# skynavga/orion-sdr

Measured on AMD Instinct MI355X. Metric: Msamples/s through WBFM demod chain (NCO+decim+FM discrim) at 1/2/4/8 MI355X, higher is better.
Workload: dtype f32; 1 GPU; C2 WBFM chain: Rotator(-f_off) -> FirDecimator(10e6, 8, 200e3, 79e3; 127 taps) -> FmQuadratureDemod(1.25e6, 75e3, 15e3) -> FirLowpass(1.25e6, 15e3, 10e3; 125 taps); channels_per_gpu=1, parallelism=channel-sharded x1, no data-path collective

## Files before the change

### orion-sdr_amd/csrc/k_wbfm.hip

```cpp
#include <algorithm>
#include <cstdlib>

#include "iir.hpp"
#include "kernels.hpp"
#include "poly.hpp"

namespace orion {
namespace {

__device__ __forceinline__ void lds_order() { asm volatile("" ::: "memory"); }

constexpr int NT = 256;
constexpr int T = kWbfmT;
constexpr int M = kWbfmM;
constexpr int Q = kWbfmQ;
using PW = Poly<M, Q, T, NT>;
static_assert(PW::NS == kWbfmNS, "staging size");
constexpr int KP = (PW::NS + 2 * NT - 1) / (2 * NT);
static_assert(2 * NT * (KP - 1) + 2 * NT - 1 >= PW::NS - 1, "staging coverage");


template <int R>
struct Fw {
  static constexpr int TW = 64 * R;
  static constexpr int NEW = M * TW;
  static constexpr int KL = NEW / 128;
  static constexpr int LR = TW + Q + 2;
  static constexpr int WIN = (R + Q) / 2;
  static constexpr int LDS_F2 = M * LR;
  static_assert(LR % 16 == 2, "row pitch = 2 mod 16 (phase-scattered b64 stores)");
  static_assert((R % 2) == 0 && NEW <= kWbfmNS, "phasor table covers the tile");
};


__device__ __forceinline__ float wave_shr1(float v, float first) {
  return __int_as_float(__builtin_amdgcn_update_dpp(__float_as_int(first), __float_as_int(v), 0x138,
                                                    0xf, 0xf, false));
}

template <int R, bool A16, bool CLAMP>
__device__ __forceinline__ void front2_load(const f2* __restrict__ x, long long n, long long porg,
                                            int l, f2 (&v)[Fw<R>::KL][2]) {
  const long long B = porg + 8 * Q;
  const f2* __restrict__ xb;
  int lo = 0, hi = 0;
  if constexpr (CLAMP) {
    constexpr long long kSat = 1LL << 30;
    lo = static_cast<int>(max(-B, -kSat));
    hi = static_cast<int>(min(max((n - 2 - B) & ~1LL, -kSat), kSat));
    xb = x + B;
  } else {
    xb = x + min(max(B, 0LL), (n - Fw<R>::NEW) & ~1LL);
  }
#pragma unroll
  for (int k = 0; k < Fw<R>::KL; ++k) {
    const int o = CLAMP ? min(max(2 * l + 128 * k, lo), hi) : 2 * l + 128 * k;
    if constexpr (A16) {
      const f4 w = __builtin_nontemporal_load(reinterpret_cast<const f4*>(xb + o));
      v[k][0] = f2{w.x, w.y};
      v[k][1] = f2{w.z, w.w};
    } else {
      v[k][0] = xb[o];
      v[k][1] = xb[o + 1];
    }
  }
}

template <int R>
__device__ __forceinline__ void front2_phase(const f4 (&w)[Fw<R>::WIN], const float (&t)[Q], f2 (&d)[R]) {
#pragma unroll
  for (int h = 0; h < Fw<R>::WIN; ++h) {
    const f2 w0 = f2{w[h].x, w[h].y}, w1 = f2{w[h].z, w[h].w};
#pragma unroll
    for (int r = 0; r < R; ++r) {
      const int q0 = r + Q - 2 * h, q1 = r + Q - 2 * h - 1;
      if (q0 >= 0 && q0 < Q) d[r] = fma2(splat2(t[q0]), w0, d[r]);
      if (q1 >= 0 && q1 < Q) d[r] = fma2(splat2(t[q1]), w1, d[r]);
    }
  }
}

template <int R>
__device__ __forceinline__ void front2_window(const f2* __restrict__ U, int l, int c, f4 (&w)[Fw<R>::WIN]) {
  const f4* row = reinterpret_cast<const f4*>(U + c * Fw<R>::LR + R * l);
#pragma unroll
  for (int h = 0; h < Fw<R>::WIN; ++h) w[h] = row[h];
}
__device__ __forceinline__ void front2_taps(const float* __restrict__ g, int c, float (&t)[Q]) {
#pragma unroll
  for (int q = 0; q < Q; ++q) t[q] = g[c * Q + q];
}

template <int R>
__device__ __forceinline__ void front2_decim(const f2* __restrict__ U, int l, const float* __restrict__ g,
                                             f2 (&d)[R]) {
#pragma unroll
  for (int r = 0; r < R; ++r) d[r] = f2{0.0f, 0.0f};
#pragma unroll 1
  for (int c = 0; c < M; ++c) {
    f4 w[Fw<R>::WIN];
    float t[Q];
    front2_window<R>(U, l, c, w);
    front2_taps(g, c, t);
    front2_phase<R>(w, t, d);
  }
}

template <int R, bool A16, bool CLAMP = false>
__global__ __launch_bounds__(64, R <= 2 ? 3 : 2) void k_wbfm_front2(const WbfmArgs a, const WbfmFrontConst C,
                                                    long long L, int wpc) {
  using G = Fw<R>;
  __shared__ __attribute__((aligned(16))) f2 U[G::LDS_F2];
  const int l = threadIdx.x;
  const int ch = blockIdx.x / wpc;
  const long long A = static_cast<long long>(blockIdx.x - ch * wpc) * L;
  const long long B = min(A + L, a.n_dec);
  if (A >= B) return;
// ... 356 lines not shown
template <int N>
struct Geo {
  static constexpr int L = 128 * N;
  static constexpr int NH = L / 2;
  static constexpr int CH = NH / 64;
  static_assert((CH & (CH - 1)) == 0 && CH >= 8, "chunk a power of two");
  __host__ __device__ static constexpr int pslot(int e) { return e + e / CH; }
  static constexpr int PSlots = pslot(NH + PB) + 1;
};

__device__ __forceinline__ void st_agent(uint32_t* p, uint32_t v) {
  __hip_atomic_store(p, v, __ATOMIC_RELAXED, __HIP_MEMORY_SCOPE_AGENT);
}
__device__ __forceinline__ uint32_t ld_agent(const uint32_t* p) {
  return __hip_atomic_load(p, __ATOMIC_RELAXED, __HIP_MEMORY_SCOPE_AGENT);
}
__device__ __forceinline__ void stores_done() { __builtin_amdgcn_s_waitcnt(0x0F70); }
__device__ __forceinline__ void publish(uint32_t* flag, uint32_t epoch, int l) {
  stores_done();
  if (l == 0) st_agent(flag, epoch);
}
__device__ __forceinline__ void wait_for(const uint32_t* flag, uint32_t epoch, int* err, uint32_t spin) {
  for (uint32_t it = 0; it < spin; ++it) {
    if (ld_agent(flag) == epoch) {
      asm volatile("" ::: "memory");
      return;
    }
    __builtin_amdgcn_s_sleep(4);
  }
  if ((threadIdx.x & 63) == 0) __hip_atomic_store(err, 1, __ATOMIC_RELAXED, __HIP_MEMORY_SCOPE_SYSTEM);
}
__device__ __forceinline__ double u2d(uint32_t lo, uint32_t hi) {
  return __longlong_as_double(static_cast<long long>((static_cast<unsigned long long>(hi) << 32) | lo));
}
}

struct FuTile {
  const WbfmArgs& a;
  const WbfmFrontConst& C;
  f2* U;
  float* Phi;
  const float* Gt;
  const f2* xc;
  const f2* hc;
  const f2* tabc;
  int ch, l, s0, s1;
  f2 corr;
  bool first;
};
struct FuPrefetch {
  const f2* xl;
  long long nl, porg;
  bool on;
};

namespace g8 {
constexpr int PCH = 91;
constexpr int LRS = 2 * PCH;
constexpr int LDS_F2 = M * LRS;
__host__ __device__ constexpr int pchunk(int c) { return 5 * (c >> 2) + (c & 3); }
__host__ __device__ constexpr int slot(int i) { return 2 * pchunk(i >> 1) + (i & 1); }
static_assert(slot(fu::G::TW + Q) < LRS && pchunk(fu::G::TW / 2) == 80, "row geometry");
__device__ __forceinline__ int group(int l) {
  const int i = l & 31;
  const bool a = i < 4 || (i >= 12 && i < 16) || (i >= 20 && i < 28);
  return (l >> 5) * 2 + (a ? 0 : 1);
}
__device__ __forceinline__ int prev_lane(int l) {
  const int row = l >> 4, lp = l & 15;
  return row == 0 ? 47 + lp : row == 2 ? lp : row == 1 ? 32 + lp : 16 + lp;
}
__device__ __forceinline__ int first_out(int l) {
  const int row = l >> 4;
  return 8 * (l & 15) + 2 * (row == 0 ? 0 : row == 2 ? 1 : row == 1 ? 2 : 3);
}
template <bool FIRST, bool ORD>
__device__ __forceinline__ void phase(const f2* __restrict__ U, int c, int lp, const float* __restrict__ Gt,
                                      f2 (&d)[8]) {
  const f4* __restrict__ row = reinterpret_cast<const f4*>(U + c * LRS) + 5 * lp;
  const f4* __restrict__ tq = reinterpret_cast<const f4*>(Gt + c * Q);
  f4 w[12];
  float t[Q];
  if constexpr (ORD) {
#pragma unroll
    for (int q4 = Q / 4 - 1; q4 >= 0; --q4) {
      const f4 u = tq[q4];
      t[4 * q4] = u.x;
      t[4 * q4 + 1] = u.y;
      t[4 * q4 + 2] = u.z;
      t[4 * q4 + 3] = u.w;
    }
#pragma unroll
    for (int h = 0; h < 12; ++h) w[h] = row[5 * (h >> 2) + (h & 3)];
  } else {
#pragma unroll
    for (int h = 0; h < 12; ++h) w[h] = row[5 * (h >> 2) + (h & 3)];
#pragma unroll
    for (int q4 = 0; q4 < Q / 4; ++q4) {
      const f4 u = tq[q4];
      t[4 * q4] = u.x;
      t[4 * q4 + 1] = u.y;
      t[4 * q4 + 2] = u.z;
      t[4 * q4 + 3] = u.w;
    }
  }
#pragma unroll
  for (int qi = 0; qi < Q; ++qi) {
    const int q = ORD ? Q - 1 - qi : qi;
#pragma unroll
    for (int r = 0; r < 8; ++r) {
      const int m = r + Q - q;
      const f4& wc = w[m >> 1];
      const f2 xv = (m & 1) ? f2{wc.z, wc.w} : f2{wc.x, wc.y};
      if (FIRST && qi == 0) {
        d[r] = splat2(t[q]) * xv;
      } else {
        d[r] = fma2(splat2(t[q]), xv, d[r]);
      }
    }
  }
}
}

template <bool A16, bool CLAMP>
__device__ __forceinline__ void fu_tile8(const FuTile& T, int n, long long porg, long long jd0,
                                         const f2 (&ph)[8][2], f2 (&v)[8][2], const FuPrefetch& pf, f2 Sv,
                                         f2& carry, float* __restrict__ phit, int svi) {
  using G = fu::G;
  f2* __restrict__ U = T.U;
  const int l = T.l;
  const int hc = l & 7, hh = l >> 3;
  f4 hw = f4{0, 0, 0, 0};
  f2 hq = f2{0, 0};
  if (n > 0) {
    hw = *reinterpret_cast<const f4*>(U + hc * g8::LRS + 2 * (80 + g8::pchunk(hh)));
    if (l < 7) hq = U[(l + 1) * g8::LRS + g8::slot(G::TW + Q)];
  }
  const bool bnd = porg < 0 || porg + 8LL * (G::TW + Q) > T.a.n;
#pragma unroll
  for (int k = 0; k < G::KL; ++k) {
    U[T.s0 + 20 * k] = cmul_rot_pk(v[k][0], ph[k][0]);
    U[T.s1 + 20 * k] = cmul_rot_pk(v[k][1], ph[k][1]);
    if (k % 4 == 3) asm volatile("" ::: "memory");
  }
  asm volatile("" ::: "memory");
  if (n > 0) {
    const f2 y0 = cmul(f2{hw.x, hw.y}, T.corr), y1 = cmul(f2{hw.z, hw.w}, T.corr);
    *reinterpret_cast<f4*>(U + hc * g8::LRS + 2 * g8::pchunk(hh)) = f4{y0.x, y0.y, y1.x, y1.y};
    if (l < 7) U[(l + 1) * g8::LRS + g8::slot(Q)] = cmul(hq, T.corr);
  }
  front2_load<2, A16, CLAMP>(pf.xl, pf.nl, pf.porg, l, v);
  if (bnd) {
    lds_order();
#pragma unroll 1
    for (int p = (n == 0 ? 0 : 8 * Q) + l; p < 8 * (G::TW + Q); p += 64) {
      const long long Pp = porg + p;
      if (!CLAMP || Pp < 0 || Pp >= T.a.n || p < 8 * Q) {
        const int c = (-p) & 7;
        U[c * g8::LRS + g8::slot((p + c) / 8)] = cmul_rot(load_hist(T.xc, T.a.n, T.hc, kWbfmHist, Pp), T.tabc[p]);
      }
    }
  }
  lds_order();
  const int g = g8::group(l), lp = l & 15;
  f2 d[8];
  g8::phase<true, true>(U, 2 * g, lp, T.Gt, d);
  asm volatile("" ::: "memory");
  g8::phase<false, true>(U, 2 * g + 1, lp, T.Gt, d);
  f2 K[4];
#pragma unroll
  for (int i = 0; i < 4; ++i) {
    const auto sx = __builtin_amdgcn_permlane16_swap(__float_as_uint(d[i].x), __float_as_uint(d[i + 4].x), false, false);
    const auto sy = __builtin_amdgcn_permlane16_swap(__float_as_uint(d[i].y), __float_as_uint(d[i + 4].y), false, false);
    K[i] = f2{__uint_as_float(sx[0]), __uint_as_float(sy[0])} + f2{__uint_as_float(sx[1]), __uint_as_float(sy[1])};
  }
  f2 F[2];
#pragma unroll
  for (int i = 0; i < 2; ++i) {
    const auto sx = __builtin_amdgcn_permlane32_swap(__float_as_uint(K[i].x), __float_as_uint(K[i + 2].x), false, false);
    const auto sy = __builtin_amdgcn_permlane32_swap(__float_as_uint(K[i].y), __float_as_uint(K[i + 2].y), false, false);
    F[i] = f2{__uint_as_float(sx[0]), __uint_as_float(sy[0])} + f2{__uint_as_float(sx[1]), __uint_as_float(sy[1])};
  }
  const f2 S = f2{__int_as_float(__builtin_amdgcn_readlane(__float_as_int(Sv.x), svi)),
                  __int_as_float(__builtin_amdgcn_readlane(__float_as_int(Sv.y), svi))};
  F[0] = cmul(F[0], S);
  F[1] = cmul(F[1], S);
  if (n == 0 && !T.first) {
    f2 acc = f2{0.0f, 0.0f};
#pragma unroll
    for (int t2 = 0; t2 < 2; ++t2) {
      const int k = 2 * l + t2, c = k & 7, q = k >> 3;
      acc = fma2(splat2(T.Gt[c * Q + q]), U[c * g8::LRS + g8::slot(15 - q)], acc);
    }
#pragma unroll
    for (int off = 32; off >= 1; off >>= 1)
      acc += f2{__shfl_xor(acc.x, off, 64), __shfl_xor(acc.y, off, 64)};
    carry = cmul(acc, S);
  }
  const int src = g8::prev_lane(l);
  f2 pv = f2{__shfl(F[1].x, src, 64), __shfl(F[1].y, src, 64)};
  if (l == 0) pv = carry;
  const int j0 = g8::first_out(l);
  *reinterpret_cast<f2*>(phit + j0) = f2{fm_disc_pk_rcp(F[0], pv, T.C.k), fm_disc_pk_rcp(F[1], F[0], T.C.k)};
  carry = f2{__int_as_float(__builtin_amdgcn_readlane(__float_as_int(F[1].x), 63)),
             __int_as_float(__builtin_amdgcn_readlane(__float_as_int(F[1].y), 63))};
  const WbfmArgs& a = T.a;
  if (jd0 <= a.n_dec - 1 && a.n_dec - 1 < jd0 + G::TW) {
    const int rl = static_cast<int>(a.n_dec - 1 - jd0);
    float* co = a.carry_out + T.ch * kWbfmCarry;
#pragma unroll
    for (int r = 0; r < 2; ++r)
      if (j0 + r == rl) {
        co[4] = F[r].x;
        co[5] = F[r].y;
        co[6] = 0.0f;
        co[7] = 0.0f;
      }
#pragma unroll
    for (int t2 = 0; t2 < kWbfmHist / 64; ++t2) {
      const int t = l + 64 * t2;
      a.hist_out[T.ch * kWbfmHist + t] = load_hist(T.xc, a.n, T.hc, kWbfmHist, a.n - kWbfmHist + t);
    }
  }
}

struct FuRange {
  int r, ch, wl;
  long long A, B;
  int Lr;
  bool first, last;
};
__device__ __forceinline__ FuPrefetch fu_origin(const WbfmArgs& a, const FuRange& g) {
  const bool tiny = a.n < 2;
  FuPrefetch p;
  p.xl = tiny ? a.hist_in + g.ch * kWbfmHist : a.x + g.ch * a.x_stride;
  p.nl = tiny ? kWbfmHist : a.n;
  p.porg = 8LL * (g.A - Q);
  p.on = true;
  return p;
}

constexpr int kSegPrioQ16 = 9;
namespace sg {
constexpr int NS = 8;
using Y = fu::Geo<NS>;
constexpr int L = Y::L;
constexpr int CH = Y::CH;
constexpr int WBytes = (Y::PSlots * 8 > L * 4) ? Y::PSlots * 8 : L * 4;
constexpr int kSegSlot = kSeg4Slot;

__device__ __forceinline__ double uni(double v) {
  const long long b = __double_as_longlong(v);
  const int lo = __builtin_amdgcn_readfirstlane(static_cast<int>(b));
  const int hi = __builtin_amdgcn_readfirstlane(static_cast<int>(b >> 32));
  return __longlong_as_double((static_cast<long long>(hi) << 32) | static_cast<unsigned int>(lo));
}

typedef const __attribute__((address_space(4))) double* cmat_t;
__device__ __forceinline__ cmat_t mats_of(const WbfmFusedConst& Bc) {
  const double* p = Bc.mats;
  asm volatile("" : "+s"(p));
  return (cmat_t)(p);
}
template <int S>
__device__ __forceinline__ void matvec_c(cmat_t M, const double (&x)[S], double (&y)[S]) {
#pragma unroll
  for (int i = 0; i < S; ++i)
#pragma unroll
    for (int j = 0; j < S; ++j) y[i] = __builtin_fma(M[i * S + j], x[j], y[i]);
}
__device__ __forceinline__ void iir16(const WbfmFusedConst& Bc, const float* __restrict__ Phi, int l,
                                      const double (&sw)[4], f2 (&xs)[CH], f2 (&ef)[4], double (&send)[4]) {
#pragma unroll
  for (int i = 0; i < CH; i += 4) {
    const f4 u = *reinterpret_cast<const f4*>(Phi + 16 * l + i);
    const f4 w = *reinterpret_cast<const f4*>(Phi + 16 * l + 8 + i);
    xs[i] = f2{u.x, w.x};
    xs[i + 1] = f2{u.y, w.y};
    xs[i + 2] = f2{u.z, w.z};
    xs[i + 3] = f2{u.w, w.w};
  }
  lds_order();
  const Biquad2 bq{splat2(Bc.b0), splat2(Bc.b1), splat2(Bc.b2), splat2(Bc.a1), splat2(Bc.a2)};
  f2 z[4] = {f2{0, 0}, f2{0, 0}, f2{0, 0}, f2{0, 0}};
#pragma unroll
  for (int i = 0; i < CH; ++i) (void)bq.lp4(z, xs[i]);
  double zE[4], q[4];
#pragma unroll
  for (int k = 0; k < 4; ++k) {
    zE[k] = z[k].x;
    q[k] = z[k].y;
  }
  const cmat_t pw = mats_of(Bc);
  matvec_c<4>(pw, zE, q);
  {
    double f[4] = {0, 0, 0, 0};
    matvec_c<4>(pw + 16, sw, f);
#pragma unroll
    for (int k = 0; k < 4; ++k) q[k] += l == 0 ? f[k] : 0.0;
  }
#pragma unroll 1
  for (int st = 0; st < 6; ++st) {
    const int dd = 1 << st;
    double o[4];
#pragma unroll
    for (int k = 0; k < 4; ++k) o[k] = __shfl_up(q[k], dd, 64);
    if (l >= dd) matvec_c<4>(pw + (st + 1) * 16, o, q);
  }
#pragma unroll
  for (int k = 0; k < 4; ++k) {
    const long long b = __double_as_longlong(q[k]);
    const int lo = __builtin_amdgcn_readlane(static_cast<int>(b), 63);
    const int hi = __builtin_amdgcn_readlane(static_cast<int>(b >> 32), 63);
    send[k] = __longlong_as_double((static_cast<long long>(hi) << 32) | static_cast<unsigned int>(lo));
  }
  double eE[4], eO[4];
#pragma unroll
  for (int k = 0; k < 4; ++k) {
    const double o = __shfl_up(q[k], 1, 64);
    eE[k] = l == 0 ? sw[k] : o;
    eO[k] = zE[k];
  }
  matvec_c<4>(pw, eE, eO);
#pragma unroll
  for (int k = 0; k < 4; ++k) ef[k] = f2{static_cast<float>(eE[k]), static_cast<float>(eO[k])};
}

__device__ __forceinline__ void zs_only16(const WbfmFusedConst& Bc, const float* Phi, float* tmp, int l,
                                          double (&sw)[4], float (&hout)[2]) {
  const double zero[4] = {0, 0, 0, 0};
  f2 xs[CH], ef[4];
  iir16(Bc, Phi, l, zero, xs, ef, sw);
  const Biquad2 bq{splat2(Bc.b0), splat2(Bc.b1), splat2(Bc.b2), splat2(Bc.a1), splat2(Bc.a2)};
  int to = 16 * (l - 56);
  asm volatile("" : "+v"(to));
  float* __restrict__ tl = tmp + to;
#pragma unroll
  for (int i = 0; i < CH; ++i) {
    const f2 f = bq.lp4(ef, xs[i]);
    if (l >= 56) {
      tl[i] = f.x;
      tl[8 + i] = f.y;
    }
  }
  lds_order();
  hout[0] = tmp[l];
  hout[1] = tmp[l + 64];
  lds_order();
}

__host__ __device__ constexpr int pe(int e) { return e + ((e >> 7) << 3); }
constexpr int kFpN = pe(128 + 1024 + 16) + 8;
#ifndef ORION_WBFM_EXACT_FIR
#define ORION_WBFM_EXACT_FIR 0
#endif
#if ORION_WBFM_EXACT_FIR
__host__ __device__ constexpr int pf(int e) { return e + 4 * (e >> 6); }
constexpr int kTxOff = pf(128 + 1024 + 16) * 4;
#else
constexpr int kTxOff = 2 * kFpN * 2;
#endif
static_assert(kTxOff % 16 == 0 && kTxOff + 128 * 4 <= WBytes, "f planes + exact history fit the sub-range region");
typedef _Float16 h8 __attribute__((ext_vector_type(8)));
__device__ __forceinline__ _Float16 hi16(float x) { return static_cast<_Float16>(x); }
__device__ __forceinline__ _Float16 lo16(float x, _Float16 h) { return static_cast<_Float16>(x - static_cast<float>(h)); }

template <int CTRL>
__device__ __forceinline__ float dpp_max(float v) {
  return fmaxf(v, __int_as_float(__builtin_amdgcn_update_dpp(0, __float_as_int(v), CTRL, 0xf, 0xf, false)));
}
__device__ __forceinline__ float wave_max(float v) {
  v = dpp_max<0xB1>(v);
  v = dpp_max<0x4E>(v);
  v = dpp_max<0x141>(v);
  v = dpp_max<0x140>(v);
  const auto r16 = __builtin_amdgcn_permlane16_swap(__float_as_uint(v), __float_as_uint(v), false, false);
  v = fmaxf(__uint_as_float(r16[0]), __uint_as_float(r16[1]));
  const auto r32 = __builtin_amdgcn_permlane32_swap(__float_as_uint(v), __float_as_uint(v), false, false);
  return fmaxf(__uint_as_float(r32[0]), __uint_as_float(r32[1]));
}

__device__ __forceinline__ void publish_end(const WbfmArgs& a, int r, const double (&sw)[4], const float (&hist)[2],
                                            int l) {
  uint32_t* slot = a.hand + static_cast<long long>(r) * kSegSlot;
  if (l < 8) {
    const int kk = l >> 1;
    const double v8 = kk == 0 ? sw[0] : kk == 1 ? sw[1] : kk == 2 ? sw[2] : sw[3];
    const unsigned long long b = static_cast<unsigned long long>(__double_as_longlong(v8));
    fu::st_agent(slot + 2 + l, (l & 1) ? static_cast<uint32_t>(b >> 32) : static_cast<uint32_t>(b));
  }
  fu::st_agent(slot + 16 + l, __float_as_uint(hist[0]));
  fu::st_agent(slot + 16 + 64 + l, __float_as_uint(hist[1]));
  fu::publish(a.flags + 3LL * r, a.epoch, l);
}

__device__ __forceinline__ void back(const WbfmArgs& a, const WbfmFusedConst& Bc, int ch, long long A0, int Lr,
                                     bool chan_last, const float* Phi, void* Pv, const uint32_t* __restrict__ Aw,
                                     int l, double (&sw)[4], float (&hist)[2], int publish_r = -1,
                                     int trace_r = -1) {
  const Biquad2 bq{splat2(Bc.b0), splat2(Bc.b1), splat2(Bc.b2), splat2(Bc.a1), splat2(Bc.a2)};
  _Float16* __restrict__ Fh = static_cast<_Float16*>(Pv);
  _Float16* __restrict__ Fl = Fh + kFpN;
  float* __restrict__ Tx = reinterpret_cast<float*>(static_cast<unsigned char*>(Pv) + kTxOff);
  f2 xs[CH];
  {
    f2 ef[4];
    double send[4];
    iir16(Bc, Phi, l, sw, xs, ef, send);
    if (trace_r >= 0) fu::trace(a, trace_r, 10);
    const int jl = Lr - 1;
    float cap[4] = {0, 0, 0, 0};
    bool have = false;
#pragma unroll
    for (int i = 0; i < CH; ++i) {
      const int j = 16 * l + i;
      const f2 f = bq.lp4(ef, xs[i]);
      xs[i] = f2{j < Lr ? f.x : 0.0f, j + 8 < Lr ? f.y : 0.0f};
      const int te = j - Lr + 128;
      if (te >= 0 && te < 128) Tx[te] = f.x;
      if (te + 8 >= 0 && te + 8 < 128) Tx[te + 8] = f.y;
      if (chan_last) {
        if (j == jl) {
#pragma unroll
          for (int k = 0; k < 4; ++k) cap[k] = ef[k].x;
          have = true;
        }
        if (j + 8 == jl) {
#pragma unroll
          for (int k = 0; k < 4; ++k) cap[k] = ef[k].y;
          have = true;
        }
      }
    }
    if (have) {
      float* co = a.carry_out + ch * kWbfmCarry;
#pragma unroll
      for (int k = 0; k < 4; ++k) co[k] = cap[k];
    }
    const int lend = Lr >= L ? 63 : max(0, (Lr >> 4) - 1);
#pragma unroll
    for (int k = 0; k < 4; ++k)
      sw[k] = static_cast<double>(__int_as_float(__builtin_amdgcn_readlane(__float_as_int(ef[k].y), lend)));
  }
  if (Lr < 128) {
#pragma unroll
    for (int r2 = 0; r2 < 2; ++r2) {
      const int t = l + 64 * r2 - Lr;
      if (t >= 0) Tx[t] = hist[r2];
    }
  }
#if ORION_WBFM_EXACT_FIR
  const int sf = 0;
  {
    float* __restrict__ Fp = static_cast<float*>(Pv);
    const int e0 = pf(128 + 16 * l);
    *reinterpret_cast<f4*>(Fp + e0) = f4{xs[0].x, xs[1].x, xs[2].x, xs[3].x};
    *reinterpret_cast<f4*>(Fp + e0 + 4) = f4{xs[4].x, xs[5].x, xs[6].x, xs[7].x};
    *reinterpret_cast<f4*>(Fp + e0 + 8) = f4{xs[0].y, xs[1].y, xs[2].y, xs[3].y};
    *reinterpret_cast<f4*>(Fp + e0 + 12) = f4{xs[4].y, xs[5].y, xs[6].y, xs[7].y};
#pragma unroll
    for (int r2 = 0; r2 < 2; ++r2) Fp[pf(l + 64 * r2)] = hist[r2];
    if (l < 4) *reinterpret_cast<f4*>(Fp + pf(128 + 1024 + 4 * l)) = f4{0, 0, 0, 0};
  }
#else
  float mx = fmaxf(fabsf(hist[0]), fabsf(hist[1]));
#pragma unroll
  for (int i = 0; i < CH; ++i) mx = fmaxf(mx, fmaxf(fabsf(xs[i].x), fabsf(xs[i].y)));
  mx = wave_max(mx);
  const int sf = __builtin_amdgcn_readfirstlane(min(100, 15 - __builtin_amdgcn_frexp_expf(mx)));
  {
    typedef _Float16 h2 __attribute__((ext_vector_type(2)));
    const int e0 = pe(128 + 16 * l);
#pragma unroll
    for (int i = 0; i < CH; i += 2) {
      h2 eh, el, oh, ol;
#pragma unroll
      for (int u = 0; u < 2; ++u) {
        const float fe = __builtin_amdgcn_ldexpf(xs[i + u].x, sf), fo = __builtin_amdgcn_ldexpf(xs[i + u].y, sf);
        eh[u] = hi16(fe);
        el[u] = lo16(fe, eh[u]);
        oh[u] = hi16(fo);
        ol[u] = lo16(fo, oh[u]);
      }
      *reinterpret_cast<h2*>(Fh + e0 + i) = eh;
      *reinterpret_cast<h2*>(Fl + e0 + i) = el;
      *reinterpret_cast<h2*>(Fh + e0 + 8 + i) = oh;
      *reinterpret_cast<h2*>(Fl + e0 + 8 + i) = ol;
    }
  }
#pragma unroll
  for (int r2 = 0; r2 < 2; ++r2) {
    const int e = pe(l + 64 * r2);
    const float x = __builtin_amdgcn_ldexpf(hist[r2], sf);
    const _Float16 h = hi16(x);
    Fh[e] = h;
    Fl[e] = lo16(x, h);
  }
  if (l < 2) {
    const h8 z = h8{0, 0, 0, 0, 0, 0, 0, 0};
    *reinterpret_cast<h8*>(Fh + pe(128 + 1024 + 8 * l)) = z;
    *reinterpret_cast<h8*>(Fl + pe(128 + 1024 + 8 * l)) = z;
  }
#endif
  lds_order();
#pragma unroll
  for (int r2 = 0; r2 < 2; ++r2) hist[r2] = Tx[l + 64 * r2];
  if (publish_r >= 0) publish_end(a, publish_r, sw, hist, l);
  if (chan_last) {
#pragma unroll
    for (int r2 = 0; r2 < 2; ++r2) a.carry_out[ch * kWbfmCarry + 8 + l + 64 * r2] = hist[r2];
  }
  if (trace_r >= 0) fu::trace(a, trace_r, 11);
  {
    const int J = l & 15, kg = l >> 4;
    typedef float f4v __attribute__((ext_vector_type(4)));
    f4v acc[4];
#pragma unroll
    for (int g = 0; g < 4; ++g) acc[g] = f4v{0.0f, 0.0f, 0.0f, 0.0f};
#if ORION_WBFM_EXACT_FIR
    {
      const float* __restrict__ Fp = static_cast<const float*>(Pv);
      const float* __restrict__ At = reinterpret_cast<const float*>(Aw);
      const int I = l & 15;
#pragma unroll 4
      for (int st = 0; st < 40; ++st) {
        const float av = At[I - 4 * st - kg + 159];
        const int p = pf(16 * J + 4 * st + kg);
        float b[4];
#pragma unroll
        for (int g = 0; g < 4; ++g) b[g] = Fp[p + 272 * g];
#pragma unroll
        for (int g = 0; g < 4; ++g) acc[g] = __builtin_amdgcn_mfma_f32_16x16x4f32(av, b[g], acc[g], 0, 0, 0);
      }
    }
#else
    const int I = l & 15;
#pragma unroll 1
    for (int st = 0; st < 5; ++st) {
      h8 ah, al;
      {
        const int o = 32 * st + 8 * kg - I - 1, p = o & 1;
// ... 4 lines not shown
        ah = __builtin_bit_cast(h8, vh);
        al = __builtin_bit_cast(h8, vl);
      }
      h8 bh[4], bl[4];
#pragma unroll
      for (int g = 0; g < 4; ++g) {
        const int e = pe(256 * g + 16 * J + 32 * st + 8 * kg);
        bh[g] = *reinterpret_cast<const h8*>(Fh + e);
        bl[g] = *reinterpret_cast<const h8*>(Fl + e);
      }
#pragma unroll
      for (int g = 0; g < 4; ++g) acc[g] = __builtin_amdgcn_mfma_f32_16x16x32_f16(ah, bh[g], acc[g], 0, 0, 0);
#pragma unroll
      for (int g = 0; g < 4; ++g) acc[g] = __builtin_amdgcn_mfma_f32_16x16x32_f16(ah, bl[g], acc[g], 0, 0, 0);
#pragma unroll
      for (int g = 0; g < 4; ++g) acc[g] = __builtin_amdgcn_mfma_f32_16x16x32_f16(al, bh[g], acc[g], 0, 0, 0);
      asm volatile("" ::: "memory");
      if (trace_r >= 0 && st == 0) fu::trace(a, trace_r, 13);
    }
#endif
    if (trace_r >= 0) fu::trace(a, trace_r, 14);
    float* __restrict__ y = a.y + ch * a.y_stride + A0;
    const float ys = __builtin_amdgcn_ldexpf(Bc.tscale, -sf);
    if (Lr == L && (reinterpret_cast<uintptr_t>(y) & 15) == 0) {
#pragma unroll
      for (int g = 0; g < 4; ++g)
        *reinterpret_cast<float4*>(y + 256 * g + 16 * J + 4 * kg) =
            float4{acc[g][0] * ys, acc[g][1] * ys, acc[g][2] * ys, acc[g][3] * ys};
    } else {
#pragma unroll
      for (int g = 0; g < 4; ++g)
#pragma unroll
        for (int r = 0; r < 4; ++r) {
          const int j = 256 * g + 16 * J + 4 * kg + r;
          if (j < Lr) y[j] = acc[g][r] * ys;
        }
    }
  }
  lds_order();
  if (trace_r >= 0) fu::trace(a, trace_r, 12);
}

}

template <bool A16, bool CLAMP>
__global__ __launch_bounds__(64, 2) void k_wbfm_seg(const WbfmArgs a, const WbfmFrontConst C,
                                                    const WbfmFusedConst Bc, int spc, int S) {
  using G = fu::G;
  constexpr int TW = G::TW;
  __shared__ __attribute__((aligned(16))) f2 U[g8::LDS_F2];
  __shared__ __attribute__((aligned(16))) unsigned char wreg[sg::WBytes];
  __shared__ __attribute__((aligned(16))) float Gt[128];
  __shared__ __attribute__((aligned(16))) uint32_t Aw[kAudFragBytes / 4];
  float* Phi = reinterpret_cast<float*>(wreg);
  f2* P = reinterpret_cast<f2*>(wreg);
  const int l = threadIdx.x & 63;
  Gt[l] = C.g[l];
  Gt[l + 64] = C.g[l + 64];
  {
    const uint32_t* __restrict__ aw = static_cast<const uint32_t*>(a.afrag);
#pragma unroll
    for (int i = 0; i < kAudFragBytes / 4 / 64; ++i) Aw[l + 64 * i] = aw[l + 64 * i];
  }
  FuRange g;
  g.r = blockIdx.x;
  g.ch = g.r / spc;
  g.wl = g.r - g.ch * spc;
  g.A = static_cast<long long>(g.wl) * S;
  g.B = min(g.A + S, a.n_dec);
  g.Lr = static_cast<int>(g.B - g.A);
  g.first = g.wl == 0;
  g.last = g.B == a.n_dec;
  const bool late = blockIdx.x >= (gridDim.x >> 1);
  const int nsub = (g.Lr + sg::L - 1) / sg::L;
  const int ntiles = nsub * sg::NS;
  uint32_t* const myslot = a.hand + static_cast<long long>(g.r) * sg::kSegSlot;
  fu::trace(a, g.r, 0);

  const FuPrefetch org = fu_origin(a, g);
  f2 va[G::KL][2];
  front2_load<2, A16, CLAMP>(org.xl, org.nl, org.porg, l, va);
  const f2* __restrict__ tabc = a.tab + static_cast<long long>(g.ch) * kWbfmNS;
  const f2* __restrict__ xc = a.x + g.ch * a.x_stride;
  const f2* __restrict__ hc = a.hist_in + g.ch * kWbfmHist;
  const f2 cn = tabc[G::NEW];
  const int c0 = (-2 * l) & 7, c1 = (-2 * l - 1) & 7;
  const FuTile T{a, C, U, Phi, Gt, xc, hc, tabc, g.ch, l, c0 * g8::LRS + g8::slot((8 * Q + 2 * l + c0) / 8),
                 c1 * g8::LRS + g8::slot((8 * Q + 2 * l + 1 + c1) / 8), f2{cn.x, -cn.y}, g.first};
  long long porg = org.porg;
  {
    const long long P0 = porg + 2 * l;
    const long long hi = (org.nl & ~1LL) - 2;
    const long long Pc = P0 < 0 ? 0 : (P0 > hi ? hi : P0);
    const f2 x0 = org.xl[Pc], x1 = org.xl[Pc + 1];
    const f4 th = *reinterpret_cast<const f4*>(tabc + 2 * l);
    U[c0 * g8::LRS + g8::slot((2 * l + c0) / 8)] = cmul_rot(x0, f2{th.x, th.y});
    U[c1 * g8::LRS + g8::slot((2 * l + 1 + c1) / 8)] = cmul_rot(x1, f2{th.z, th.w});
  }
  {
    const long long Pm = max(porg - (l & 7), 0LL);
    const f2 xm = xc[Pm];
    const f2 tc = tabc[l & 7];
    if (!g.first && l >= 1 && l < 8) U[l * g8::LRS] = cmul_rot(xm, f2{tc.x, -tc.y});
  }
  f2 Sv = f2{0, 0};
  f2 carry = f2{0.0f, 0.0f};
  if (g.first) {
    const float* ci = a.carry_in + g.ch * kWbfmCarry;
    carry = f2{ci[4], ci[5]};
  }
  double sw[4] = {0, 0, 0, 0};
  float hist[2] = {0, 0};
  const FuPrefetch dummy{org.xl, org.nl, -8LL * Q, true};

#pragma unroll 1
  for (int sub = 0, n = 0; sub < nsub; ++sub) {
    f2 ph[G::KL][2];
    {
      const f4 tv = *reinterpret_cast<const f4*>(tabc + 8 * Q + 2 * l);
      const f2 tb0 = f2{tv.x, tv.y}, tb1 = f2{tv.z, tv.w};
#pragma unroll
      for (int k = 0; k < G::KL; ++k) {
        const f2 ek = tabc[128 * k];
        ph[k][0] = cmul(tb0, ek);
        ph[k][1] = cmul(tb1, ek);
      }
    }
    const long long A0 = g.A + static_cast<long long>(sub) * sg::L;
    const int Lr = static_cast<int>(min(static_cast<long long>(sg::L), g.B - A0));
#pragma unroll 1
    for (int tin = 0; tin < sg::NS; ++tin, ++n, porg += G::NEW) {
      if ((16 * n < kSegPrioQ16 * ntiles) == late) __builtin_amdgcn_s_setprio(1);
      else __builtin_amdgcn_s_setprio(0);
      if ((n & 63) == 0)
        Sv = phasor_q64(static_cast<uint64_t>(a.k0 + porg + 1 + static_cast<long long>(l) * G::NEW),
                        a.step[g.ch]);
      const long long jd0 = g.A + static_cast<long long>(n) * TW;
      const FuPrefetch p0 = n + 1 < ntiles ? FuPrefetch{org.xl, org.nl, porg + G::NEW, true} : dummy;
      fu_tile8<A16, CLAMP>(T, n, porg, jd0, ph, va, p0, Sv, carry, Phi + TW * tin, n & 63);
    }
    lds_order();
    if (sub == 0) {
      f4* gs = reinterpret_cast<f4*>(myslot + kFuSlot);
#pragma unroll
      for (int i = 0; i < sg::L / 256; ++i) gs[l + 64 * i] = *reinterpret_cast<const f4*>(Phi + 4 * (l + 64 * i));
      sg::zs_only16(Bc, Phi, Phi, l, sw, hist);
      if (nsub == 1 && !g.last) sg::publish_end(a, g.r, sw, hist, l);
    } else {
      const bool lastsub = sub == nsub - 1;
      if (sub <= 3) fu::trace(a, g.r, 3 + sub);
      sg::back(a, Bc, g.ch, A0, Lr, g.last && lastsub, Phi, P, Aw, l, sw, hist, lastsub && !g.last ? g.r : -1,
               sub == 1 ? g.r : -1);
      if (sub <= 3) fu::trace(a, g.r, 6 + sub);
    }
  }
  fu::trace(a, g.r, 1);
  const f4* gs = reinterpret_cast<const f4*>(myslot + kFuSlot);
  f4 u[sg::L / 256];
#pragma unroll
  for (int i = 0; i < sg::L / 256; ++i) u[i] = __builtin_nontemporal_load(gs + l + 64 * i);
  if (g.first) {
    const float* __restrict__ ci = a.carry_in + g.ch * kWbfmCarry;
#pragma unroll
    for (int k = 0; k < 4; ++k) sw[k] = ci[k];
    hist[0] = ci[8 + l];
    hist[1] = ci[8 + 64 + l];
  } else {
    fu::wait_for(a.flags + 3LL * (g.r - 1), a.epoch, a.err, a.spin);
    const uint32_t* ps = a.hand + static_cast<long long>(g.r - 1) * sg::kSegSlot;
#pragma unroll
    for (int k = 0; k < 4; ++k) sw[k] = sg::uni(fu::u2d(fu::ld_agent(ps + 2 + 2 * k), fu::ld_agent(ps + 3 + 2 * k)));
    hist[0] = __uint_as_float(fu::ld_agent(ps + 16 + l));
    hist[1] = __uint_as_float(fu::ld_agent(ps + 16 + 64 + l));
  }
#pragma unroll
  for (int i = 0; i < sg::L / 256; ++i) *reinterpret_cast<f4*>(Phi + 4 * (l + 64 * i)) = u[i];
  lds_order();
  fu::trace(a, g.r, 2);
  sg::back(a, Bc, g.ch, g.A, min(sg::L, g.Lr), g.last && nsub == 1, Phi, P, Aw, l, sw, hist);
  fu::trace(a, g.r, 3);
}

}

namespace {

constexpr int kFrontR = 2;

struct Front2Plan {
  int grid, wpc;
  long long L;
};
template <int R>
Front2Plan front2_plan(long long n_dec, int nch, int ncu) {
  using G = Fw<R>;
  int per_cu = std::min<int>((160 * 1024) / static_cast<int>(G::LDS_F2 * sizeof(f2)), R <= 2 ? 12 : 8);
  per_cu = std::max(4, per_cu & ~3);
  const long long slots = static_cast<long long>(per_cu) * ncu;
  const long long tiles = static_cast<long long>(nch) * ((n_dec + G::TW) / G::TW);
  const long long N = std::max<long long>(1, (tiles + slots - 1) / slots);
  Front2Plan p;
  p.L = N * G::TW - 1;
  p.wpc = static_cast<int>((n_dec + p.L - 1) / p.L);
  p.grid = p.wpc * nch;
  return p;
}

template <int R>
void launch_front2(bool a16, long long n_dec, int nch, int ncu, const WbfmArgs& a,
                   const WbfmFrontConst& f, hipStream_t s) {
  const Front2Plan fp = front2_plan<R>(n_dec, nch, ncu);
  if (a.n < 2LL * Fw<R>::NEW) {
    if (a16) k_wbfm_front2<R, true, true><<<fp.grid, 64, 0, s>>>(a, f, fp.L, fp.wpc);
    else k_wbfm_front2<R, false, true><<<fp.grid, 64, 0, s>>>(a, f, fp.L, fp.wpc);
  } else {
    if (a16) k_wbfm_front2<R, true><<<fp.grid, 64, 0, s>>>(a, f, fp.L, fp.wpc);
    else k_wbfm_front2<R, false><<<fp.grid, 64, 0, s>>>(a, f, fp.L, fp.wpc);
  }
}

}

long long wbfm_seg_slots(long long n_dec, int nch) {
  return static_cast<long long>(nch) * ((n_dec + kSgL - 1) / kSgL) + 1;
}

void launch_wbfm_seg(const WbfmArgs& a, const WbfmFrontConst& f, const WbfmFusedConst& b, int nch,
                     int max_segments, hipStream_t s) {
  static_assert(sg::L == kSgL, "sub-range geometry");
  if (a.n_dec <= 0 || nch <= 0) return;
  const int cap = resident_per_cu(reinterpret_cast<const void*>(k_wbfm_seg<true, false>), 64) * device_cus();
  const long long capx = max_segments > 0 ? max_segments : cap;
// ... 32 lines not shown
```

Before: 516,300 Msamples/s.

## Stage IIR scan matrices in LDS, hoist tile bounds checks, use immediate-offset loads

The IIR scan matrices move from constant (scalar) memory into an LDS array, and the prefix-scan loop is unrolled with next-step matrices preloaded and DPP/permlane shifts replacing the shuffles. The per-tile boundary and end-tile checks are now computed once before the loop. Interior prefetch loads use fixed immediate offsets from a precomputed base pointer. Full segments take a fast path without per-element bounds checks and write wider vector stores for the f16 split outputs. Together these aim to cut address arithmetic, scalar-cache stalls and branching, at the cost of extra LDS and more code paths.

```diff
diff --git a/orion-sdr_amd/csrc/k_wbfm.hip b/orion-sdr_amd/csrc/k_wbfm.hip
--- a/orion-sdr_amd/csrc/k_wbfm.hip
+++ b/orion-sdr_amd/csrc/k_wbfm.hip
@@ -63,6 +63,19 @@
       v[k][0] = xb[o];
       v[k][1] = xb[o + 1];
     }
+  }
+}
+
+template <int R>
+__device__ __forceinline__ void front2_load_at(const f2* __restrict__ xb, int l, f2 (&v)[Fw<R>::KL][2]) {
+  static_assert(Fw<R>::KL == 8, "immediates -4096 .. 3072");
+  const char* __restrict__ sb = reinterpret_cast<const char*>(xb) + 4096;
+  const unsigned vo = 16u * static_cast<unsigned>(l);
+#pragma unroll
+  for (int k = 0; k < Fw<R>::KL; ++k) {
+    const f4 w = __builtin_nontemporal_load(reinterpret_cast<const f4*>((sb + (1024 * k - 4096)) + vo));
+    v[k][0] = f2{w.x, w.y};
+    v[k][1] = f2{w.z, w.w};
   }
 }
 
@@ -525,6 +538,7 @@
   const f2* xl;
   long long nl, porg;
   bool on;
+  const f2* xb;
 };
 
 namespace g8 {
@@ -598,7 +612,7 @@
 template <bool A16, bool CLAMP>
 __device__ __forceinline__ void fu_tile8(const FuTile& T, int n, long long porg, long long jd0,
                                          const f2 (&ph)[8][2], f2 (&v)[8][2], const FuPrefetch& pf, f2 Sv,
-                                         f2& carry, float* __restrict__ phit, int svi) {
+                                         f2& carry, float* __restrict__ phit, int svi, bool bnd, bool endt) {
   using G = fu::G;
   f2* __restrict__ U = T.U;
   const int l = T.l;
@@ -609,7 +623,6 @@
     hw = *reinterpret_cast<const f4*>(U + hc * g8::LRS + 2 * (80 + g8::pchunk(hh)));
     if (l < 7) hq = U[(l + 1) * g8::LRS + g8::slot(G::TW + Q)];
   }
-  const bool bnd = porg < 0 || porg + 8LL * (G::TW + Q) > T.a.n;
 #pragma unroll
   for (int k = 0; k < G::KL; ++k) {
     U[T.s0 + 20 * k] = cmul_rot_pk(v[k][0], ph[k][0]);
@@ -622,7 +635,8 @@
     *reinterpret_cast<f4*>(U + hc * g8::LRS + 2 * g8::pchunk(hh)) = f4{y0.x, y0.y, y1.x, y1.y};
     if (l < 7) U[(l + 1) * g8::LRS + g8::slot(Q)] = cmul(hq, T.corr);
   }
-  front2_load<2, A16, CLAMP>(pf.xl, pf.nl, pf.porg, l, v);
+  if constexpr (A16 && !CLAMP) front2_load_at<2>(pf.xb, l, v);
+  else front2_load<2, A16, CLAMP>(pf.xl, pf.nl, pf.porg, l, v);
   if (bnd) {
     lds_order();
 #pragma unroll 1
@@ -678,7 +692,7 @@
   carry = f2{__int_as_float(__builtin_amdgcn_readlane(__float_as_int(F[1].x), 63)),
              __int_as_float(__builtin_amdgcn_readlane(__float_as_int(F[1].y), 63))};
   const WbfmArgs& a = T.a;
-  if (jd0 <= a.n_dec - 1 && a.n_dec - 1 < jd0 + G::TW) {
+  if (endt) {
     const int rl = static_cast<int>(a.n_dec - 1 - jd0);
     float* co = a.carry_out + T.ch * kWbfmCarry;
 #pragma unroll
@@ -710,6 +724,7 @@
   p.nl = tiny ? kWbfmHist : a.n;
   p.porg = 8LL * (g.A - Q);
   p.on = true;
+  p.xb = p.xl + min(max(p.porg + 8 * Q, 0LL), max((p.nl - fu::G::NEW) & ~1LL, 0LL));
   return p;
 }
 
@@ -729,21 +744,65 @@
   return __longlong_as_double((static_cast<long long>(hi) << 32) | static_cast<unsigned int>(lo));
 }
 
-typedef const __attribute__((address_space(4))) double* cmat_t;
-__device__ __forceinline__ cmat_t mats_of(const WbfmFusedConst& Bc) {
-  const double* p = Bc.mats;
-  asm volatile("" : "+s"(p));
-  return (cmat_t)(p);
+typedef double d2 __attribute__((ext_vector_type(2)));
+typedef const __attribute__((address_space(3))) double* lmat_t;
+typedef const __attribute__((address_space(3))) d2* lmat2_t;
+__device__ __forceinline__ lmat_t mats_of(const double* Ms) {
+  unsigned o = static_cast<unsigned>(reinterpret_cast<uintptr_t>((lmat_t)(Ms)));
+  asm volatile("" : "+v"(o));
+  return (lmat_t)(static_cast<uintptr_t>(o));
+}
+__device__ __forceinline__ void mat_lds(lmat_t Ms, int k, double (&m)[16]) {
+  const lmat2_t p = (lmat2_t)(Ms + 16 * k);
+#pragma unroll
+  for (int i = 0; i < 8; ++i) {
+    const d2 v = p[i];
+    m[2 * i] = v.x;
+    m[2 * i + 1] = v.y;
+  }
 }
 template <int S>
-__device__ __forceinline__ void matvec_c(cmat_t M, const double (&x)[S], double (&y)[S]) {
+__device__ __forceinline__ void matvec_r(const double (&M)[S * S], const double (&x)[S], double (&y)[S]) {
 #pragma unroll
   for (int i = 0; i < S; ++i)
 #pragma unroll
     for (int j = 0; j < S; ++j) y[i] = __builtin_fma(M[i * S + j], x[j], y[i]);
 }
-__device__ __forceinline__ void iir16(const WbfmFusedConst& Bc, const float* __restrict__ Phi, int l,
-                                      const double (&sw)[4], f2 (&xs)[CH], f2 (&ef)[4], double (&send)[4]) {
+template <int D>
+__device__ __forceinline__ double lane_up(double v) {
+  if constexpr (D == 1 || D == 32) {
+    const long long b = __double_as_longlong(v);
+    int lo = static_cast<int>(b), hi = static_cast<int>(b >> 32);
+    if constexpr (D == 1) {
+      lo = __builtin_amdgcn_update_dpp(lo, lo, 0x138, 0xf, 0xf, false);
+      hi = __builtin_amdgcn_update_dpp(hi, hi, 0x138, 0xf, 0xf, false);
+    } else {
+      const unsigned ul = static_cast<unsigned>(lo), uh = static_cast<unsigned>(hi);
+      lo = static_cast<int>(__builtin_amdgcn_permlane32_swap(ul, ul, false, false)[0]);
+      hi = static_cast<int>(__builtin_amdgcn_permlane32_swap(uh, uh, false, false)[0]);
+    }
+    return __longlong_as_double((static_cast<long long>(hi) << 32) | static_cast<unsigned int>(lo));
+  } else {
+    return __shfl_up(v, D, 64);
+  }
+}
+template <int ST>
+__device__ __forceinline__ void scan_step(lmat_t Ms, int l, double (&Mc)[16], double (&q)[4]) {
+  constexpr int dd = 1 << ST;
+  double Mn[16];
+  lds_order();
+  mat_lds(Ms, ST < 5 ? ST + 2 : 0, Mn);
+  lds_order();
+  double o[4];
+#pragma unroll
+  for (int k = 0; k < 4; ++k) o[k] = lane_up<dd>(q[k]);
+  if (l >= dd) matvec_r<4>(Mc, o, q);
+#pragma unroll
+  for (int i = 0; i < 16; ++i) Mc[i] = Mn[i];
+}
+__device__ __forceinline__ void iir16(const WbfmFusedConst& Bc, const double* __restrict__ Msg,
+                                      const float* __restrict__ Phi, int l, const double (&sw)[4], f2 (&xs)[CH],
+                                      f2 (&ef)[4], double (&send)[4]) {
 #pragma unroll
   for (int i = 0; i < CH; i += 4) {
     const f4 u = *reinterpret_cast<const f4*>(Phi + 16 * l + i);
@@ -753,6 +812,10 @@
     xs[i + 2] = f2{u.z, w.z};
     xs[i + 3] = f2{u.w, w.w};
   }
+  const lmat_t Ms = mats_of(Msg);
+  double M8[16], Mc[16];
+  mat_lds(Ms, 0, M8);
+  mat_lds(Ms, 1, Mc);
   lds_order();
   const Biquad2 bq{splat2(Bc.b0), splat2(Bc.b1), splat2(Bc.b2), splat2(Bc.a1), splat2(Bc.a2)};
   f2 z[4] = {f2{0, 0}, f2{0, 0}, f2{0, 0}, f2{0, 0}};
@@ -764,22 +827,19 @@
     zE[k] = z[k].x;
     q[k] = z[k].y;
   }
-  const cmat_t pw = mats_of(Bc);
-  matvec_c<4>(pw, zE, q);
+  matvec_r<4>(M8, zE, q);
   {
     double f[4] = {0, 0, 0, 0};
-    matvec_c<4>(pw + 16, sw, f);
+    matvec_r<4>(Mc, sw, f);
 #pragma unroll
     for (int k = 0; k < 4; ++k) q[k] += l == 0 ? f[k] : 0.0;
   }
-#pragma unroll 1
-  for (int st = 0; st < 6; ++st) {
-    const int dd = 1 << st;
-    double o[4];
-#pragma unroll
-    for (int k = 0; k < 4; ++k) o[k] = __shfl_up(q[k], dd, 64);
-    if (l >= dd) matvec_c<4>(pw + (st + 1) * 16, o, q);
-  }
+  scan_step<0>(Ms, l, Mc, q);
+  scan_step<1>(Ms, l, Mc, q);
+  scan_step<2>(Ms, l, Mc, q);
+  scan_step<3>(Ms, l, Mc, q);
+  scan_step<4>(Ms, l, Mc, q);
+  scan_step<5>(Ms, l, Mc, q);
 #pragma unroll
   for (int k = 0; k < 4; ++k) {
     const long long b = __double_as_longlong(q[k]);
@@ -790,31 +850,31 @@
   double eE[4], eO[4];
 #pragma unroll
   for (int k = 0; k < 4; ++k) {
-    const double o = __shfl_up(q[k], 1, 64);
+    const double o = lane_up<1>(q[k]);
     eE[k] = l == 0 ? sw[k] : o;
     eO[k] = zE[k];
   }
-  matvec_c<4>(pw, eE, eO);
+  matvec_r<4>(Mc, eE, eO);
 #pragma unroll
   for (int k = 0; k < 4; ++k) ef[k] = f2{static_cast<float>(eE[k]), static_cast<float>(eO[k])};
 }
 
-__device__ __forceinline__ void zs_only16(const WbfmFusedConst& Bc, const float* Phi, float* tmp, int l,
-                                          double (&sw)[4], float (&hout)[2]) {
+__device__ __forceinline__ void zs_only16(const WbfmFusedConst& Bc, const double* __restrict__ Ms, const float* Phi,
+                                          float* tmp, int l, double (&sw)[4], float (&hout)[2]) {
   const double zero[4] = {0, 0, 0, 0};
   f2 xs[CH], ef[4];
-  iir16(Bc, Phi, l, zero, xs, ef, sw);
+  iir16(Bc, Ms, Phi, l, zero, xs, ef, sw);
   const Biquad2 bq{splat2(Bc.b0), splat2(Bc.b1), splat2(Bc.b2), splat2(Bc.a1), splat2(Bc.a2)};
-  int to = 16 * (l - 56);
-  asm volatile("" : "+v"(to));
-  float* __restrict__ tl = tmp + to;
-#pragma unroll
-  for (int i = 0; i < CH; ++i) {
-    const f2 f = bq.lp4(ef, xs[i]);
-    if (l >= 56) {
-      tl[i] = f.x;
-      tl[8 + i] = f.y;
-    }
+#pragma unroll
+  for (int i = 0; i < CH; ++i) xs[i] = bq.lp4(ef, xs[i]);
+  if (l >= 56) {
+    int lt = l & 7;
+    asm volatile("" : "+v"(lt));
+    f4* __restrict__ tl = reinterpret_cast<f4*>(tmp + 16 * lt);
+    tl[0] = f4{xs[0].x, xs[1].x, xs[2].x, xs[3].x};
+    tl[1] = f4{xs[4].x, xs[5].x, xs[6].x, xs[7].x};
+    tl[2] = f4{xs[0].y, xs[1].y, xs[2].y, xs[3].y};
+    tl[3] = f4{xs[4].y, xs[5].y, xs[6].y, xs[7].y};
   }
   lds_order();
   hout[0] = tmp[l];
@@ -855,6 +915,7 @@
 
 __device__ __forceinline__ void publish_end(const WbfmArgs& a, int r, const double (&sw)[4], const float (&hist)[2],
                                             int l) {
+  asm volatile("" : "+v"(l));
   uint32_t* slot = a.hand + static_cast<long long>(r) * kSegSlot;
   if (l < 8) {
     const int kk = l >> 1;
@@ -867,10 +928,10 @@
   fu::publish(a.flags + 3LL * r, a.epoch, l);
 }
 
-__device__ __forceinline__ void back(const WbfmArgs& a, const WbfmFusedConst& Bc, int ch, long long A0, int Lr,
-                                     bool chan_last, const float* Phi, void* Pv, const uint32_t* __restrict__ Aw,
-                                     int l, double (&sw)[4], float (&hist)[2], int publish_r = -1,
-                                     int trace_r = -1) {
+__device__ __forceinline__ void back(const WbfmArgs& a, const WbfmFusedConst& Bc, const double* __restrict__ Ms,
+                                     int ch, long long A0, int Lr, bool chan_last, const float* Phi, void* Pv,
+                                     const uint32_t* __restrict__ Aw, int l, double (&sw)[4], float (&hist)[2],
+                                     int publish_r = -1, int trace_r = -1) {
   const Biquad2 bq{splat2(Bc.b0), splat2(Bc.b1), splat2(Bc.b2), splat2(Bc.a1), splat2(Bc.a2)};
   _Float16* __restrict__ Fh = static_cast<_Float16*>(Pv);
   _Float16* __restrict__ Fl = Fh + kFpN;
@@ -879,41 +940,60 @@
   {
     f2 ef[4];
     double send[4];
-    iir16(Bc, Phi, l, sw, xs, ef, send);
+    iir16(Bc, Ms, Phi, l, sw, xs, ef, send);
     if (trace_r >= 0) fu::trace(a, trace_r, 10);
-    const int jl = Lr - 1;
-    float cap[4] = {0, 0, 0, 0};
-    bool have = false;
-#pragma unroll
-    for (int i = 0; i < CH; ++i) {
-      const int j = 16 * l + i;
-      const f2 f = bq.lp4(ef, xs[i]);
-      xs[i] = f2{j < Lr ? f.x : 0.0f, j + 8 < Lr ? f.y : 0.0f};
-      const int te = j - Lr + 128;
-      if (te >= 0 && te < 128) Tx[te] = f.x;
-      if (te + 8 >= 0 && te + 8 < 128) Tx[te + 8] = f.y;
-      if (chan_last) {
-        if (j == jl) {
-#pragma unroll
-          for (int k = 0; k < 4; ++k) cap[k] = ef[k].x;
-          have = true;
+    if (Lr == L && !chan_last) {
+#pragma unroll
+      for (int i = 0; i < CH; ++i) xs[i] = bq.lp4(ef, xs[i]);
+      if (l >= 56) {
+        int lt = l & 7;
+        asm volatile("" : "+v"(lt));
+        f4* __restrict__ tl = reinterpret_cast<f4*>(Tx + 16 * lt);
+        tl[0] = f4{xs[0].x, xs[1].x, xs[2].x, xs[3].x};
+        tl[1] = f4{xs[4].x, xs[5].x, xs[6].x, xs[7].x};
+        tl[2] = f4{xs[0].y, xs[1].y, xs[2].y, xs[3].y};
+        tl[3] = f4{xs[4].y, xs[5].y, xs[6].y, xs[7].y};
+      }
+#pragma unroll
+      for (int k = 0; k < 4; ++k)
+        sw[k] = static_cast<double>(__int_as_float(__builtin_amdgcn_readlane(__float_as_int(ef[k].y), 63)));
+    } else {
+      const int jl = Lr - 1;
+      float cap[4] = {0, 0, 0, 0};
+      bool have = false;
+      int lg = l;
+      asm volatile("" : "+v"(lg));
+#pragma unroll
+      for (int i = 0; i < CH; ++i) {
+        const int j = 16 * lg + i;
+        const f2 f = bq.lp4(ef, xs[i]);
+        xs[i] = f2{j < Lr ? f.x : 0.0f, j + 8 < Lr ? f.y : 0.0f};
+        const int te = j - Lr + 128;
+        if (te >= 0 && te < 128) Tx[te] = f.x;
+        if (te + 8 >= 0 && te + 8 < 128) Tx[te + 8] = f.y;
+        if (chan_last) {
+          if (j == jl) {
+#pragma unroll
+            for (int k = 0; k < 4; ++k) cap[k] = ef[k].x;
+            have = true;
+          }
+          if (j + 8 == jl) {
+#pragma unroll
+            for (int k = 0; k < 4; ++k) cap[k] = ef[k].y;
+            have = true;
+          }
         }
-        if (j + 8 == jl) {
-#pragma unroll
-          for (int k = 0; k < 4; ++k) cap[k] = ef[k].y;
-          have = true;
-        }
-      }
-    }
-    if (have) {
-      float* co = a.carry_out + ch * kWbfmCarry;
-#pragma unroll
-      for (int k = 0; k < 4; ++k) co[k] = cap[k];
-    }
-    const int lend = Lr >= L ? 63 : max(0, (Lr >> 4) - 1);
-#pragma unroll
-    for (int k = 0; k < 4; ++k)
-      sw[k] = static_cast<double>(__int_as_float(__builtin_amdgcn_readlane(__float_as_int(ef[k].y), lend)));
+      }
+      if (have) {
+        float* co = a.carry_out + ch * kWbfmCarry;
+#pragma unroll
+        for (int k = 0; k < 4; ++k) co[k] = cap[k];
+      }
+      const int lend = Lr >= L ? 63 : max(0, (Lr >> 4) - 1);
+#pragma unroll
+      for (int k = 0; k < 4; ++k)
+        sw[k] = static_cast<double>(__int_as_float(__builtin_amdgcn_readlane(__float_as_int(ef[k].y), lend)));
+    }
   }
   if (Lr < 128) {
 #pragma unroll
@@ -942,24 +1022,22 @@
   mx = wave_max(mx);
   const int sf = __builtin_amdgcn_readfirstlane(min(100, 15 - __builtin_amdgcn_frexp_expf(mx)));
   {
-    typedef _Float16 h2 __attribute__((ext_vector_type(2)));
-    const int e0 = pe(128 + 16 * l);
-#pragma unroll
-    for (int i = 0; i < CH; i += 2) {
-      h2 eh, el, oh, ol;
-#pragma unroll
-      for (int u = 0; u < 2; ++u) {
-        const float fe = __builtin_amdgcn_ldexpf(xs[i + u].x, sf), fo = __builtin_amdgcn_ldexpf(xs[i + u].y, sf);
-        eh[u] = hi16(fe);
-        el[u] = lo16(fe, eh[u]);
-        oh[u] = hi16(fo);
-        ol[u] = lo16(fo, oh[u]);
-      }
-      *reinterpret_cast<h2*>(Fh + e0 + i) = eh;
-      *reinterpret_cast<h2*>(Fl + e0 + i) = el;
-      *reinterpret_cast<h2*>(Fh + e0 + 8 + i) = oh;
-      *reinterpret_cast<h2*>(Fl + e0 + 8 + i) = ol;
-    }
+    int lo = l;
+    asm volatile("" : "+v"(lo));
+    const int e0 = pe(128 + 16 * lo);
+    h8 eh, el, oh, ol;
+#pragma unroll
+    for (int i = 0; i < CH; ++i) {
+      const float fe = __builtin_amdgcn_ldexpf(xs[i].x, sf), fo = __builtin_amdgcn_ldexpf(xs[i].y, sf);
+      eh[i] = hi16(fe);
+      el[i] = lo16(fe, eh[i]);
+      oh[i] = hi16(fo);
+      ol[i] = lo16(fo, oh[i]);
+    }
+    *reinterpret_cast<h8*>(Fh + e0) = eh;
+    *reinterpret_cast<h8*>(Fh + e0 + 8) = oh;
+    *reinterpret_cast<h8*>(Fl + e0) = el;
+    *reinterpret_cast<h8*>(Fl + e0 + 8) = ol;
   }
 #pragma unroll
   for (int r2 = 0; r2 < 2; ++r2) {
@@ -1070,6 +1148,7 @@
   __shared__ __attribute__((aligned(16))) unsigned char wreg[sg::WBytes];
   __shared__ __attribute__((aligned(16))) float Gt[128];
   __shared__ __attribute__((aligned(16))) uint32_t Aw[kAudFragBytes / 4];
+  __shared__ __attribute__((aligned(16))) double Ms[kWbfmMats];
   float* Phi = reinterpret_cast<float*>(wreg);
   f2* P = reinterpret_cast<f2*>(wreg);
   const int l = threadIdx.x & 63;
@@ -1079,6 +1158,8 @@
     const uint32_t* __restrict__ aw = static_cast<const uint32_t*>(a.afrag);
 #pragma unroll
     for (int i = 0; i < kAudFragBytes / 4 / 64; ++i) Aw[l + 64 * i] = aw[l + 64 * i];
+    if (l < kWbfmMats / 2)
+      reinterpret_cast<sg::d2*>(Ms)[l] = reinterpret_cast<const sg::d2*>(Bc.mats)[l];
   }
   FuRange g;
   g.r = blockIdx.x;
@@ -1097,7 +1178,8 @@
 
   const FuPrefetch org = fu_origin(a, g);
   f2 va[G::KL][2];
-  front2_load<2, A16, CLAMP>(org.xl, org.nl, org.porg, l, va);
+  if constexpr (A16 && !CLAMP) front2_load_at<2>(org.xb, l, va);
+  else front2_load<2, A16, CLAMP>(org.xl, org.nl, org.porg, l, va);
   const f2* __restrict__ tabc = a.tab + static_cast<long long>(g.ch) * kWbfmNS;
   const f2* __restrict__ xc = a.x + g.ch * a.x_stride;
   const f2* __restrict__ hc = a.hist_in + g.ch * kWbfmHist;
@@ -1129,7 +1211,13 @@
   }
   double sw[4] = {0, 0, 0, 0};
   float hist[2] = {0, 0};
-  const FuPrefetch dummy{org.xl, org.nl, -8LL * Q, true};
+  const FuPrefetch dummy{org.xl, org.nl, -8LL * Q, true, org.xl};
+  const int nhi = static_cast<int>(
+      min(max(((a.n - 8LL * (TW + Q) - org.porg) >> 10) + 1, 0LL), static_cast<long long>(ntiles)));
+  const long long nend64 = (a.n_dec - 1 - g.A) >> 7;
+  const int nend = nend64 >= 0 && nend64 < ntiles ? static_cast<int>(nend64) : -1;
+  static_assert(G::NEW == 1024 && TW == 128, "the shifts above");
+  const f2* __restrict__ xhi = org.xl + max((org.nl - G::NEW) & ~1LL, 0LL);
 
 #pragma unroll 1
   for (int sub = 0, n = 0; sub < nsub; ++sub) {
@@ -1154,20 +1242,26 @@
         Sv = phasor_q64(static_cast<uint64_t>(a.k0 + porg + 1 + static_cast<long long>(l) * G::NEW),
                         a.step[g.ch]);
       const long long jd0 = g.A + static_cast<long long>(n) * TW;
-      const FuPrefetch p0 = n + 1 < ntiles ? FuPrefetch{org.xl, org.nl, porg + G::NEW, true} : dummy;
-      fu_tile8<A16, CLAMP>(T, n, porg, jd0, ph, va, p0, Sv, carry, Phi + TW * tin, n & 63);
+      const FuPrefetch p0 =
+          n + 1 < ntiles ? FuPrefetch{org.xl, org.nl, porg + G::NEW, true,
+                                      n + 1 < nhi ? org.xl + (porg + G::NEW + 8 * Q) : xhi}
+                         : dummy;
+      fu_tile8<A16, CLAMP>(T, n, porg, jd0, ph, va, p0, Sv, carry, Phi + TW * tin, n & 63,
+                           (g.first && n == 0) || n >= nhi, n == nend);
     }
     lds_order();
     if (sub == 0) {
-      f4* gs = reinterpret_cast<f4*>(myslot + kFuSlot);
-#pragma unroll
-      for (int i = 0; i < sg::L / 256; ++i) gs[l + 64 * i] = *reinterpret_cast<const f4*>(Phi + 4 * (l + 64 * i));
-      sg::zs_only16(Bc, Phi, Phi, l, sw, hist);
+      int lp = l;
+      asm volatile("" : "+v"(lp));
+      f4* gs = reinterpret_cast<f4*>(myslot + kFuSlot) + lp;
+#pragma unroll
+      for (int i = 0; i < sg::L / 256; ++i) gs[64 * i] = *reinterpret_cast<const f4*>(Phi + 4 * (l + 64 * i));
+      sg::zs_only16(Bc, Ms, Phi, Phi, l, sw, hist);
       if (nsub == 1 && !g.last) sg::publish_end(a, g.r, sw, hist, l);
     } else {
       const bool lastsub = sub == nsub - 1;
       if (sub <= 3) fu::trace(a, g.r, 3 + sub);
-      sg::back(a, Bc, g.ch, A0, Lr, g.last && lastsub, Phi, P, Aw, l, sw, hist, lastsub && !g.last ? g.r : -1,
+      sg::back(a, Bc, Ms, g.ch, A0, Lr, g.last && lastsub, Phi, P, Aw, l, sw, hist, lastsub && !g.last ? g.r : -1,
                sub == 1 ? g.r : -1);
       if (sub <= 3) fu::trace(a, g.r, 6 + sub);
     }
@@ -1195,7 +1289,7 @@
   for (int i = 0; i < sg::L / 256; ++i) *reinterpret_cast<f4*>(Phi + 4 * (l + 64 * i)) = u[i];
   lds_order();
   fu::trace(a, g.r, 2);
-  sg::back(a, Bc, g.ch, g.A, min(sg::L, g.Lr), g.last && nsub == 1, Phi, P, Aw, l, sw, hist);
+  sg::back(a, Bc, Ms, g.ch, g.A, min(sg::L, g.Lr), g.last && nsub == 1, Phi, P, Aw, l, sw, hist);
   fu::trace(a, g.r, 3);
 }
 
```

Result: no change. 518,600 Msamples/s, median of 6 (+0.4%).
